# openai/whisper

Hardware: AMD Instinct MI355X
Metric: audio-seconds transcribed per wall-second (large-v3 greedy) (higher is better)
Workload: dtype f16

## Files before the change

whisper_amd/csrc/gemv.hip:

```cpp
#include "common.h"
#include "kernels.h"
#include <stdlib.h>

#ifndef WH_GEMV8_MAX_ROWS
#define WH_GEMV8_MAX_ROWS 24
#endif

namespace {

#define ISSUE_FENCE() asm volatile("" ::: "memory")

constexpr int CS = 4;

__device__ __forceinline__ float4v load_part4(const float* p) { return *(const float4v*)p; }
__device__ __forceinline__ float4v load_part4(const half_t* p) {
  const half4v h = *(const half4v*)p;
  return float4v{(float)h[0], (float)h[1], (float)h[2], (float)h[3]};
}

template <typename T> struct Pack4;
template <> struct Pack4<float> {
  static __device__ __forceinline__ void store(float* p, float a, float b, float c, float d) {
    *(float4v*)p = float4v{a, b, c, d};
  }
// ... 903 lines not shown
      sw = across_groups8_sum(sw);
#pragma unroll
      for (int rt = 0; rt < NRT; ++rt) { s1[rt] = across_groups8_sum(s1[rt]); s2[rt] = across_groups8_sum(s2[rt]); }
      if (lane < 8) {
        wsum[mw][lane] = sw;
#pragma unroll
        for (int rt = 0; rt < NRT; ++rt) { xstat[mw][rt][0][lane] = s1[rt]; xstat[mw][rt][1][lane] = s2[rt]; }
      }
    }
  }
  WH_PROBE_AT(a, wgid, 4);
  __syncthreads();
  WH_PROBE_AT(a, wgid, 5);
#pragma unroll
  for (int j = 0; j < NOUT; ++j) {
    const int o = tid + NT * j;
    const int es = o / (NRT * 64), ert = (o >> 6) % NRT, er = (o >> 3) & 7, ej = o & 7;
    const int en = blockIdx.x * fw + es * 8 + ej;
    const bool on = o < GS * NRT * 64 && ert * 8 + er < R && es * 8 + ej < fw && en < a.N;
    if (on) {
      float v = POST ? 0.f : e_bias[j];
#pragma unroll
      for (int k = 0; k < KS; ++k) v += red[es * KS + k][ert][ej][er];
      const int64_t rr = r0 + ert * 8 + er;
      const int n = en;
      if constexpr (POST) {
        float t1 = 0.f, t2 = 0.f, tw = 0.f;
#pragma unroll
        for (int k = 0; k < KS; ++k) { t1 += xstat[es * KS + k][ert][0][er]; t2 += xstat[es * KS + k][ert][1][er]; tw += wsum[es * KS + k][ej]; }
        const float invK = 1.0f / (float)K;
        const float mc = t1 * invK;
        const float var = fmaxf(__builtin_fmaf(-mc, mc, t2 * invK), 0.f);
        v = __builtin_fmaf(rsqrtf(var + 1e-5f), __builtin_fmaf(-mc, tw, v), e_bias[j]);
      }
      switch (a.epi) {
        case whk::EPI_STORE: ((half_t*)a.y)[a.y_frag ? frag_elem(rr, n, a.N) : rr * a.y_ld + n] = (half_t)v; break;
        case whk::EPI_GELU: ((half_t*)a.y)[a.y_frag ? frag_elem(rr, n, a.N) : rr * a.y_ld + n] = (half_t)gelu_erf(v); break;
        case whk::EPI_F32: ((float*)a.y)[rr * a.y_ld + n] = v; break;
        case whk::EPI_RESID: {
          const float xr = e_res[j] + v;
          a.resid[rr * a.resid_ld + n] = xr;
          if (a.xh) ((half_t*)a.xh)[frag_elem(rr, n, a.N)] = (half_t)fminf(fmaxf(xr - e_cen[j], -65504.f), 65504.f);
        } break;
        case whk::EPI_QKV: {
          const int D = a.D;
          if (n < D) ((half_t*)a.y)[rr * a.y_ld + n] = (half_t)v;
          else {
            const int64_t pos = e_pos - e_lag[j];
            if (n < 2 * D) ((half_t*)a.kcache)[rr * a.cache_bs + pos * D + (n - D)] = (half_t)v;
            else ((half_t*)a.vcache)[rr * a.cache_bs + pos * D + (n - 2 * D)] = (half_t)v;
          }
        } break;
      }
    }
  }
  WH_PROBE_AT(a, wgid, 6);
  if (a.bump && blockIdx.x == 0 && blockIdx.y == 0 && tid == 0) atomicAdd(a.bump, a.bump_by);
  if (a.bump2 && blockIdx.x == 0 && blockIdx.y == 0 && tid == 0) atomicAdd(a.bump2, 1);
}

template <int PRO, int GS, int KS, int CSm, int XW, int NRT>
hipError_t launch_gemv8_nrt(const whk::GemvArgs& a, int fw, hipStream_t stream) {
  constexpr int WAVES = GS * KS + XW;
  static_assert(WAVES <= 16, "at most 1024 threads per workgroup");
  if (fw < 1 || fw > 8 * GS) return hipErrorInvalidValue;
  whk::g_form = WH_FORM_NAME("gemv8/%s/gs%d/ks%d/xw%d/rt%d", PRO == whk::PRO_PLAIN ? "plain" : PRO == whk::PRO_LN ? "LN" : PRO == whk::PRO_LN_POST ? "LNpost" :
                             CSm == 2 ? "combine2" : CSm == 3 ? "combine3" : "combine4", GS, KS, XW, NRT);
  const int nblk = a.K / 64;
  const int nu = (nblk + KS - 1) / KS;
  dim3 grid((a.N + fw - 1) / fw, (a.R + 8 * NRT - 1) / (8 * NRT)), block(WAVES * 64);
  if constexpr (KS == 2) {
    if (nu > 10) return hipErrorInvalidValue;
    hipLaunchKernelGGL((gemv8_kernel<PRO, GS, KS, 10, CSm, XW, NRT>), grid, block, 0, stream, a, fw);
  } else {
    if (nu <= 3) hipLaunchKernelGGL((gemv8_kernel<PRO, GS, KS, 3, CSm, XW, NRT>), grid, block, 0, stream, a, fw);
    else if (nu <= 5) hipLaunchKernelGGL((gemv8_kernel<PRO, GS, KS, 5, CSm, XW, NRT>), grid, block, 0, stream, a, fw);
    else return hipErrorInvalidValue;
  }
  return hipGetLastError();
}

template <int PRO, int GS, int KS, int CSm, int XW>
hipError_t launch_gemv8_cfg(const whk::GemvArgs& a, int fw, hipStream_t stream) {
  if (a.R <= 8) return launch_gemv8_nrt<PRO, GS, KS, CSm, XW, 1>(a, fw, stream);
  if (a.R <= 16) return launch_gemv8_nrt<PRO, GS, KS, CSm, XW, 2>(a, fw, stream);
  if constexpr (GS * KS + XW < 16) {
    if (a.R > 24) return launch_gemv8_nrt<PRO, GS, KS, CSm, XW, 6>(a, fw, stream);
  }
  return launch_gemv8_nrt<PRO, GS, KS, CSm, XW, 3>(a, fw, stream);
}

static int gemv8_fw(int N, int gs) {
  static int ncu = 256;
  int fw = (N + ncu - 1) / ncu;
  if (fw > 8 * gs) fw = 8 * gs;
  if (fw < 4) fw = N < 8 ? N : 8 < 8 * gs ? 8 : 8 * gs;
  return fw;
}

static int gemv8_slots(int N, int pro) {
  const int ngroups = (N + 7) / 8;
  if (pro == whk::PRO_LN) return ngroups >= 600 ? 3 : ngroups >= 400 ? 2 : 1;
  return 1;
}

template <int PRO, int CSm>
hipError_t launch_gemv8_pro(const whk::GemvArgs& a, hipStream_t stream) {
  const int nblk = a.K / 64, gs = gemv8_slots(a.N, PRO), fw = gemv8_fw(a.N, gs);
  if constexpr (PRO == whk::PRO_LN_POST) {
    return a.R <= 16 ? launch_gemv8_nrt<PRO, 1, 4, CSm, 0, 2>(a, fw, stream) : launch_gemv8_nrt<PRO, 1, 4, CSm, 0, 3>(a, fw, stream);
  } else if constexpr (PRO == whk::PRO_PLAIN) {
    if (nblk > 20) {
      whk::GemvArgs b = a;
      b.w_ordered = !WH_DEV_FLAG("WH_GEMV8_W_OPERAND_ORDER");
      return launch_gemv8_cfg<PRO, 1, 16, CSm, 0>(b, fw, stream);
    }
    return launch_gemv8_cfg<PRO, 1, 4, CSm, 0>(a, fw, stream);
  } else {
    if constexpr (PRO == whk::PRO_LN) {
      if (gs == 3 && a.R > 8 && !WH_DEV_FLAG("WH_GEMV8_LN3_KS4")) {
        if (a.R <= 16) return launch_gemv8_nrt<PRO, 3, 2, CSm, 8, 2>(a, fw, stream);
        return launch_gemv8_nrt<PRO, 3, 2, CSm, 8, 3>(a, fw, stream);
      }
      if (gs == 3) return launch_gemv8_cfg<PRO, 3, 4, CSm, 4>(a, fw, stream);
      if (gs == 2) return launch_gemv8_cfg<PRO, 2, 4, CSm, 8>(a, fw, stream);
    }
    return launch_gemv8_cfg<PRO, 1, 4, CSm, 8>(a, fw, stream);
  }
}

bool gemv8_applies(const whk::GemvArgs& a) {
  if (WH_DEV_FLAG("WH_GEMV_DOT2")) return false;
  if (a.variant != 0 || a.R < 1 || a.R > 96 || a.K % 64 != 0) return false;
  const int nblk = a.K / 64;
  if (nblk > 20 && (a.pro != whk::PRO_PLAIN || (nblk + 15) / 16 > 5)) return false;
  if (a.xh && a.epi == whk::EPI_RESID && (a.N % 64 != 0 || !a.xc)) return false;
  if (a.epi == whk::EPI_F32 && a.N > 16384) return false;
  if ((int64_t)a.N * a.K >= (1ll << 31)) return false;
  switch (a.pro) {
    case whk::PRO_PLAIN: return a.x_ld % 8 == 0 && (int64_t)a.R * a.x_ld < (1ll << 30);
    case whk::PRO_LN: return a.ln_folded && a.xf_ld % 4 == 0 && (int64_t)a.R * a.xf_ld < (1ll << 29);
    case whk::PRO_LN_POST: return a.ln_folded && a.R > 8 && a.R <= WH_GEMV8_MAX_ROWS && a.R <= 24 && a.epi != whk::EPI_RESID;
    case whk::PRO_COMBINE:
      return a.K == a.H * 64 && a.H <= 20 && a.splits >= 2 && a.splits <= 4 && (int64_t)a.R * a.H * a.splits * 64 < (1ll << 29);
  }
  return false;
}

hipError_t launch_gemv8(const whk::GemvArgs& a, hipStream_t stream) {
  if (a.pro == whk::PRO_PLAIN) return launch_gemv8_pro<whk::PRO_PLAIN, 1>(a, stream);
  if (a.pro == whk::PRO_LN) return launch_gemv8_pro<whk::PRO_LN, 1>(a, stream);
  if (a.pro == whk::PRO_LN_POST) return a.xh ? launch_gemv8_pro<whk::PRO_LN_POST, 1>(a, stream) : hipErrorInvalidValue;
  if (a.pro == whk::PRO_COMBINE && a.splits == 2) return launch_gemv8_pro<whk::PRO_COMBINE, 2>(a, stream);
  if (a.pro == whk::PRO_COMBINE && a.splits == 3) return launch_gemv8_pro<whk::PRO_COMBINE, 3>(a, stream);
  if (a.pro == whk::PRO_COMBINE && a.splits == 4) return launch_gemv8_pro<whk::PRO_COMBINE, 4>(a, stream);
  return hipErrorInvalidValue;
}

template <int NFT>
__global__ __launch_bounds__(1024) void gemv_rows48_kernel(whk::GemvArgs a) {
  extern __shared__ __attribute__((aligned(16))) char smem[];
  pin_kernargs(a);
  constexpr int WAVES = 16, RT = 48, KSP = WAVES / NFT, J = 5, NU = (40 + KSP - 1) / KSP;
  const int K = a.K, nks = K / 32;
  half_t* xs = (half_t*)smem;
  float* red = (float*)smem;
  const int tid = threadIdx.x, lane = tid & 63;
  const int wave = __builtin_amdgcn_readfirstlane(tid >> 6);
  const int ft = wave % NFT, ksp = wave / NFT;
  const int i16 = lane & 15, g4 = lane >> 4;
  const int n0 = blockIdx.x * (NFT * 16);
  const int R = a.R;

  float4v v[3][J];
#pragma unroll
  for (int i = 0; i < 3; ++i) {
    const int r = wave + WAVES * i;
    const float* src = a.xf + (int64_t)(r < R ? r : 0) * a.xf_ld;
#pragma unroll
    for (int j = 0; j < J; ++j) {
      int k = (j * 64 + lane) * 4; if (k > K - 4) k = K - 4;
      v[i][j] = *(const float4v*)(src + k);
    }
  }
  ISSUE_FENCE();
  half8v w[NU];
  {
    int n = n0 + ft * 16 + i16; if (n > a.N - 1) n = a.N - 1;
    const half_t* base = (const half_t*)a.W + (int64_t)n * K + g4 * 8;
#pragma unroll
    for (int u = 0; u < NU; ++u) {
      int st = ksp + KSP * u; if (st > nks - 1) st = nks - 1;
      w[u] = __builtin_nontemporal_load((const half8v*)(base + st * 32));
    }
  }
  ISSUE_FENCE();
  int e_pos = 0;
  if (a.epi == whk::EPI_QKV) e_pos = load_agent_int(a.d_pos);
  float e_bias[(NFT * 768 + 1023) / 1024];
#pragma unroll
  for (int q = 0; q < (NFT * 768 + 1023) / 1024; ++q) {
    const int o = tid + q * 1024;
    int n = n0 + ((o >> 8) / 3) * 16 + (o & 15); if (n > a.N - 1) n = a.N - 1;
    e_bias[q] = a.bias ? a.bias[n] : 0.f;
  }

  {
    const float invK = 1.0f / (float)K;
#pragma unroll
    for (int i = 0; i < 3; ++i) {
      const int r = wave + WAVES * i;
      float sum = 0.f;
#pragma unroll
      for (int j = 0; j < J; ++j) {
        const float t = (v[i][j][0] + v[i][j][1]) + (v[i][j][2] + v[i][j][3]);
        sum += ((j * 64 + lane) * 4 < K) ? t : 0.f;
      }
      const float mean = wave_sum(sum) * invK;
      float ss = 0.f;
#pragma unroll
      for (int j = 0; j < J; ++j) {
        if ((j * 64 + lane) * 4 < K) {
#pragma unroll
          for (int e = 0; e < 4; ++e) { const float d = v[i][j][e] - mean; ss = __builtin_fmaf(d, d, ss); }
        }
      }
      const float rstd = r < R ? rsqrtf(wave_sum(ss) * invK + 1e-5f) : 0.f;
      half_t* xr = xs + (size_t)r * K;
#pragma unroll
      for (int j = 0; j < J; ++j) {
        const int k = (j * 64 + lane) * 4;
        if (k < K)
          Pack4<half_t>::store(xr + ((((k >> 3) ^ (r & 15)) << 3) | (k & 7)), (v[i][j][0] - mean) * rstd,
                               (v[i][j][1] - mean) * rstd, (v[i][j][2] - mean) * rstd, (v[i][j][3] - mean) * rstd);
      }
    }
  }
  __syncthreads();

  float4v acc[3];
#pragma unroll
  for (int rt = 0; rt < 3; ++rt) acc[rt] = float4v{0.f, 0.f, 0.f, 0.f};
#pragma unroll
  for (int u = 0; u < NU; ++u) {
    const int st = ksp + KSP * u;
    if (st < nks) {
#pragma unroll
      for (int rt = 0; rt < 3; ++rt) {
        const half8v xf = *(const half8v*)(xs + (size_t)(rt * 16 + i16) * K + (((st * 4 + g4) ^ i16) << 3));
        acc[rt] = __builtin_amdgcn_mfma_f32_16x16x32_f16(w[u], xf, acc[rt], 0, 0, 0);
      }
    }
  }
  __syncthreads();
#pragma unroll
  for (int rt = 0; rt < 3; ++rt) *(float4v*)(red + ((((ksp * NFT + ft) * 3 + rt) * 16 + i16) * 16 + g4 * 4)) = acc[rt];
  __syncthreads();

#pragma unroll
  for (int q = 0; q < (NFT * 768 + 1023) / 1024; ++q) {
    const int o = tid + q * 1024;
    if (o >= NFT * 768) continue;
    const int f = o & 15, j = (o >> 4) & 15, rt = (o >> 8) % 3, oft = (o >> 8) / 3;
    const int row = rt * 16 + j, n = n0 + oft * 16 + f;
    if (row >= R || n >= a.N) continue;
    float val = e_bias[q];
#pragma unroll
    for (int k = 0; k < KSP; ++k) val += red[((((k * NFT + oft) * 3 + rt) * 16 + j) * 16) + f];
    const int64_t rr = row;
    switch (a.epi) {
      case whk::EPI_STORE: ((half_t*)a.y)[rr * a.y_ld + n] = (half_t)val; break;
      case whk::EPI_GELU: ((half_t*)a.y)[rr * a.y_ld + n] = (half_t)gelu_erf(val); break;
      case whk::EPI_QKV: {
        const int D = a.D;
        if (n < D) ((half_t*)a.y)[rr * a.y_ld + n] = (half_t)val;
        else {
          const int64_t pos = e_pos - (a.lag ? a.lag[row] : 0);
          if (n < 2 * D) ((half_t*)a.kcache)[rr * a.cache_bs + pos * D + (n - D)] = (half_t)val;
          else ((half_t*)a.vcache)[rr * a.cache_bs + pos * D + (n - 2 * D)] = (half_t)val;
        }
      } break;
      default: break;
    }
  }
  if (a.bump && blockIdx.x == 0 && tid == 0) atomicAdd(a.bump, a.bump_by);
  if (a.bump2 && blockIdx.x == 0 && tid == 0) atomicAdd(a.bump2, 1);
}

bool rows48_applies(const whk::GemvArgs& a) {
  return !WH_DEV_FLAG("WH_NO_ROWS48") && a.R > WH_GEMV8_MAX_ROWS && a.R <= 48 && a.pro == whk::PRO_LN && a.ln_folded &&
         a.K % 256 == 0 && a.K <= 1280 && a.N >= 2048 && a.variant <= 0 &&
         (a.epi == whk::EPI_STORE || a.epi == whk::EPI_GELU || a.epi == whk::EPI_QKV);
}

hipError_t launch_rows48(const whk::GemvArgs& a, hipStream_t stream) {
  whk::g_form = "rows48";
  const size_t lds = (size_t)48 * a.K * 2 > 49152 ? (size_t)48 * a.K * 2 : 49152;
  static whk::LdsAttr attr2;
  { hipError_t e = whk::raise_dynamic_lds(attr2, (const void*)gemv_rows48_kernel<2>, 160 * 1024); if (e != hipSuccess) return e; }
  hipLaunchKernelGGL((gemv_rows48_kernel<2>), dim3((a.N + 31) / 32), dim3(1024), lds, stream, a);
  return hipGetLastError();
}

__global__ __launch_bounds__(1024) void gemv_rows48_stream_kernel(whk::GemvArgs a) {
  extern __shared__ __attribute__((aligned(16))) char smem[];
  pin_kernargs(a);
  constexpr int WAVES = 16, J = 5, NB = 20;
  const int K = a.K, nks = K / 32;
  half_t* xs = (half_t*)smem;
  float* gb = (float*)(smem + (size_t)48 * K * 2);
  const int tid = threadIdx.x, lane = tid & 63;
  const int wave = __builtin_amdgcn_readfirstlane(tid >> 6);
  const int i16 = lane & 15, g4 = lane >> 4;
  const int R = a.R;
  const int ntiles = (a.N + 15) / 16;

  float4v v[3][J];
#pragma unroll
  for (int i = 0; i < 3; ++i) {
    const int r = wave + WAVES * i;
    const float* src = a.xf + (int64_t)(r < R ? r : 0) * a.xf_ld;
#pragma unroll
    for (int j = 0; j < J; ++j) {
      int k = (j * 64 + lane) * 4; if (k > K - 4) k = K - 4;
      v[i][j] = *(const float4v*)(src + k);
    }
  }
  for (int k = tid * 4; k < K; k += 4096) {
    *(float4v*)(gb + k) = *(const float4v*)(a.ln_w + k);
    *(float4v*)(gb + K + k) = *(const float4v*)(a.ln_b + k);
  }
  __syncthreads();
  {
    const float invK = 1.0f / (float)K;
#pragma unroll
    for (int i = 0; i < 3; ++i) {
      const int r = wave + WAVES * i;
      float sum = 0.f;
#pragma unroll
      for (int j = 0; j < J; ++j) {
        const float t = (v[i][j][0] + v[i][j][1]) + (v[i][j][2] + v[i][j][3]);
        sum += ((j * 64 + lane) * 4 < K) ? t : 0.f;
      }
      const float mean = wave_sum(sum) * invK;
      float ss = 0.f;
#pragma unroll
      for (int j = 0; j < J; ++j) {
        if ((j * 64 + lane) * 4 < K) {
#pragma unroll
          for (int e = 0; e < 4; ++e) { const float d = v[i][j][e] - mean; ss = __builtin_fmaf(d, d, ss); }
        }
      }
      const float rstd = rsqrtf(wave_sum(ss) * invK + 1e-5f);
      half_t* xr = xs + (size_t)r * K;
#pragma unroll
      for (int j = 0; j < J; ++j) {
        const int k = (j * 64 + lane) * 4;
        if (k < K) {
          const float4v w4 = *(const float4v*)(gb + k), b4 = *(const float4v*)(gb + K + k);
          half_t* dst = xr + ((((k >> 3) ^ (r & 15)) << 3) | (k & 7));
          if (r < R)
            Pack4<half_t>::store(dst, (v[i][j][0] - mean) * rstd * w4[0] + b4[0], (v[i][j][1] - mean) * rstd * w4[1] + b4[1],
                                 (v[i][j][2] - mean) * rstd * w4[2] + b4[2], (v[i][j][3] - mean) * rstd * w4[3] + b4[3]);
          else
            Pack4<half_t>::store(dst, 0.f, 0.f, 0.f, 0.f);
        }
      }
    }
  }
  __syncthreads();

  for (int tile = blockIdx.x * WAVES + wave; tile < ntiles; tile += gridDim.x * WAVES) {
    int n = tile * 16 + i16; if (n > a.N - 1) n = a.N - 1;
    const half_t* base = (const half_t*)a.W + (int64_t)n * K + g4 * 8;
    float4v acc[3];
#pragma unroll
    for (int rt = 0; rt < 3; ++rt) acc[rt] = float4v{0.f, 0.f, 0.f, 0.f};
    for (int st0 = 0; st0 < nks; st0 += NB) {
      half8v w[NB];
#pragma unroll
      for (int u = 0; u < NB; ++u) {
        int st = st0 + u; if (st > nks - 1) st = nks - 1;
        w[u] = __builtin_nontemporal_load((const half8v*)(base + st * 32));
      }
#pragma unroll
      for (int u = 0; u < NB; ++u) {
        const int st = st0 + u;
        if (st < nks) {
#pragma unroll
          for (int rt = 0; rt < 3; ++rt) {
            const half8v xf = *(const half8v*)(xs + (size_t)(rt * 16 + i16) * K + (((st * 4 + g4) ^ i16) << 3));
            acc[rt] = __builtin_amdgcn_mfma_f32_16x16x32_f16(w[u], xf, acc[rt], 0, 0, 0);
          }
        }
      }
    }
#pragma unroll
    for (int rt = 0; rt < 3; ++rt) {
      const int row = rt * 16 + i16;
      if (row < R) {
        float* y = (float*)a.y + (int64_t)row * a.y_ld + tile * 16 + g4 * 4;
#pragma unroll
        for (int e = 0; e < 4; ++e)
          if (tile * 16 + g4 * 4 + e < a.N) y[e] = acc[rt][e];
      }
    }
  }
  if (a.bump && blockIdx.x == 0 && tid == 0) atomicAdd(a.bump, a.bump_by);
  if (a.bump2 && blockIdx.x == 0 && tid == 0) atomicAdd(a.bump2, 1);
}

bool rows48_stream_applies(const whk::GemvArgs& a) {
  return !WH_DEV_FLAG("WH_NO_ROWS48") && a.R > 16 && a.R <= 48 && a.pro == whk::PRO_LN && a.epi == whk::EPI_F32 && !a.bias &&
         a.K % 256 == 0 && a.K <= 1280 && a.N >= 16384 && a.variant <= 0;
}

hipError_t launch_rows48_stream(const whk::GemvArgs& a, hipStream_t stream) {
  whk::g_form = "rows48_stream";
  const size_t lds = (size_t)48 * a.K * 2 + (size_t)2 * a.K * 4;
  static whk::LdsAttr attr;
  { hipError_t e = whk::raise_dynamic_lds(attr, (const void*)gemv_rows48_stream_kernel, 160 * 1024); if (e != hipSuccess) return e; }
  const int ntiles = (a.N + 15) / 16;
  int wgs = (ntiles + 15) / 16;
  if (wgs > 256) wgs = 256;
  hipLaunchKernelGGL(gemv_rows48_stream_kernel, dim3(wgs), dim3(1024), lds, stream, a);
  return hipGetLastError();
}

template <typename T, int MS>
__global__ __launch_bounds__(256) void merge_partials_kernel(const T* __restrict__ part_o, const float* __restrict__ part_ml,
                                                             int S, int R, int H, T* __restrict__ out, int64_t o_ld, int o_frag) {
  const int i = blockIdx.x * 256 + threadIdx.x;
  if (i >= R * H * 16) return;
  const int r = i / (H * 16), rem = i - r * (H * 16);
  const int h = rem >> 4, d4 = rem & 15;
  const int64_t pb = (int64_t)r * H + h, ps = (int64_t)R * H;
  float2v ml[MS];
  float4v o[MS];
#pragma unroll
  for (int s = 0; s < MS; ++s) {
    const int sc = s < S ? s : S - 1;
    ml[s] = *(const float2v*)(part_ml + (pb + sc * ps) * 2);
    o[s] = load_part4(part_o + (pb + sc * ps) * 64 + d4 * 4);
  }
  float M = WH_NEG_INF;
#pragma unroll
  for (int s = 0; s < MS; ++s) { if (s >= S) ml[s] = float2v{WH_NEG_INF, 0.f}; M = fmaxf(M, ml[s][0]); }
  float w[MS], den = 0.f;
#pragma unroll
  for (int s = 0; s < MS; ++s) {
    w[s] = (ml[s][0] == WH_NEG_INF) ? 0.f : __expf(ml[s][0] - M);
    den = __builtin_fmaf(w[s], ml[s][1], den);
  }
  const float inv = 1.0f / den;
  float4v num = {0.f, 0.f, 0.f, 0.f};
#pragma unroll
  for (int s = 0; s < MS; ++s) {
    const float f = w[s] * ml[s][1] * inv;
    num[0] = __builtin_fmaf(f, o[s][0], num[0]); num[1] = __builtin_fmaf(f, o[s][1], num[1]);
    num[2] = __builtin_fmaf(f, o[s][2], num[2]); num[3] = __builtin_fmaf(f, o[s][3], num[3]);
  }
  Pack4<T>::store(out + (o_frag ? frag_elem(r, h * 64 + d4 * 4, H * 64) : (int64_t)r * o_ld + h * 64 + d4 * 4), num[0], num[1], num[2], num[3]);
}

enum class Family { refuse, gemv8, rows48, rows48_stream, rows16_mf, rt4, rt8 };

Family pick_family(const whk::GemvArgs& a, int dtype) {
  if (a.R <= 0) return Family::refuse;
  if (a.xc && a.pro != whk::PRO_LN && !(a.xh && a.epi == whk::EPI_RESID)) return Family::refuse;
  if (a.x_frag || a.y_frag || a.pro == whk::PRO_LN_POST || a.xh || a.xc) return dtype == 1 && a.R <= WH_GEMV8_MAX_ROWS && gemv8_applies(a) ? Family::gemv8 : Family::refuse;
  if (dtype != 1) return a.R <= 4 || a.K > 3072 ? Family::rt4 : Family::rt8;
  if (rows48_applies(a)) return Family::rows48;
  if (rows48_stream_applies(a)) return Family::rows48_stream;
  const bool rows16 = a.R > 8 && a.variant <= 0 && a.K % 128 == 0 && a.K <= 5120 && (a.K / 32 <= 40 || a.pro == whk::PRO_PLAIN);
  if ((a.R <= WH_GEMV8_MAX_ROWS || !rows16) && gemv8_applies(a)) return Family::gemv8;
  if (a.R <= 4) return Family::rt4;
  if (rows16) return Family::rows16_mf;
  return Family::rt8;
}

}

namespace whk {

thread_local const char* g_form = "";

hipError_t launch_gemv(const GemvArgs& a, int dtype, hipStream_t stream) {
  const Family f = pick_family(a, dtype);
  if (dtype == 1) {
    switch (f) {
      case Family::gemv8: return launch_gemv8(a, stream);
      case Family::rows48: return launch_rows48(a, stream);
      case Family::rows48_stream: return launch_rows48_stream(a, stream);
      case Family::rt4: return launch_rt<half_t, 4>(a, stream);
      case Family::rows16_mf: return launch_rows16_mf<half_t>(a, stream);
      case Family::rt8: return launch_rt<half_t, 8>(a, stream);
      case Family::refuse: break;
    }
  } else if (f == Family::rt4 || f == Family::rt8) {
    return f == Family::rt4 ? launch_rt<float, 4>(a, stream) : launch_rt<float, 8>(a, stream);
  }
  return hipErrorInvalidValue;
}

const char* gemv_family(const GemvArgs& a, int dtype) {
  static const char* const names[] = {"", "gemv8", "rows48", "rows48_stream", "rows16_mf", "rt4", "rt8"};
  return names[(int)pick_family(a, dtype)];
}

bool gemv8_will_run(int R, int N, int K, int pro) {
  GemvArgs a = {};
  a.pro = pro; a.R = R; a.N = N; a.K = K; a.x_ld = a.xf_ld = K; a.ln_folded = 1; a.splits = 2; a.H = K / 64;
  a.epi = EPI_STORE; a.y_frag = 1;
  return pick_family(a, 1) == Family::gemv8;
}

bool gemv8_ln_post_pays(int R, int N, int K) {
  GemvArgs a = {};
  a.pro = PRO_LN_POST; a.R = R; a.N = N; a.K = K; a.ln_folded = 1; a.epi = EPI_STORE;
  return pick_family(a, 1) == Family::gemv8 && gemv8_slots(N, PRO_LN) == 1 && gemv8_will_run(R, N, K, PRO_LN);
}

hipError_t launch_merge_partials(const void* part_o, const float* part_ml, int splits, int R, int H, void* out,
                                 int64_t o_ld, int dtype, hipStream_t stream, int o_frag) {
  if (splits < 1 || splits > DEC_ATTN_MAX_SPLITS || R <= 0 || H <= 0) return hipErrorInvalidValue;
  const int n = R * H * 16;
  const dim3 grid((n + 255) / 256), block(256);
  g_form = dtype == 1 ? (splits <= 4 ? "merge<half,4>" : "merge<half,16>") : (splits <= 4 ? "merge<float,4>" : "merge<float,16>");
  if (dtype == 1) {
    if (splits <= 4)
      hipLaunchKernelGGL((merge_partials_kernel<half_t, 4>), grid, block, 0, stream, (const half_t*)part_o, part_ml, splits, R, H, (half_t*)out, o_ld, o_frag);
    else
      hipLaunchKernelGGL((merge_partials_kernel<half_t, DEC_ATTN_MAX_SPLITS>), grid, block, 0, stream, (const half_t*)part_o, part_ml, splits, R, H, (half_t*)out, o_ld, o_frag);
  } else {
    if (splits <= 4)
      hipLaunchKernelGGL((merge_partials_kernel<float, 4>), grid, block, 0, stream, (const float*)part_o, part_ml, splits, R, H, (float*)out, o_ld, o_frag);
    else
      hipLaunchKernelGGL((merge_partials_kernel<float, DEC_ATTN_MAX_SPLITS>), grid, block, 0, stream, (const float*)part_o, part_ml, splits, R, H, (float*)out, o_ld, o_frag);
  }
  return hipGetLastError();
}

}
```

Before: 1177.

## Pipeline weight loads across tiles and specialize rows48 stream GEMV on K and row tiles

Templates the LN-fused rows48 streaming GEMV on K/256 and on the number of 16-row tiles (2 when R<=32), so loops are fully unrolled and one row tile of MFMA work is skipped for smaller batches. Weight loads are double-buffered in blocks of 8: the first tile's weights are requested before the LayerNorm prologue, and the next tile's weights are prefetched right after the current tile's output stores. The grid becomes up to 256 workgroups with one tile per wave interleaved, and LDS addressing is precomputed per lane. The cost is more template instantiations and higher register pressure from the two weight buffers.

```diff
diff --git a/whisper_amd/csrc/gemv.hip b/whisper_amd/csrc/gemv.hip
--- a/whisper_amd/csrc/gemv.hip
+++ b/whisper_amd/csrc/gemv.hip
@@ -1229,39 +1229,61 @@
   return hipGetLastError();
 }
 
+template <int NB, int U0 = 0, int U1 = NB>
+__device__ __forceinline__ void rows48_stream_request(half8v (&w)[NB], const half_t* base, int b) {
+#pragma unroll
+  for (int u = U0; u < U1; ++u) w[u] = __builtin_nontemporal_load((const half8v*)(base + (b * NB + u) * 32));
+}
+
+template <int NT, int NBT>
 __global__ __launch_bounds__(1024) void gemv_rows48_stream_kernel(whk::GemvArgs a) {
   extern __shared__ __attribute__((aligned(16))) char smem[];
   pin_kernargs(a);
-  constexpr int WAVES = 16, J = 5, NB = 20;
-  const int K = a.K, nks = K / 32;
+  constexpr int WAVES = 16, J = 5, NB = 8;
+  constexpr int K = 256 * NBT;
+  constexpr int E1 = NT == 2 ? 2 : 0;
   half_t* xs = (half_t*)smem;
-  float* gb = (float*)(smem + (size_t)48 * K * 2);
+  float* gb = (float*)(smem + (size_t)(16 * NT) * K * 2);
   const int tid = threadIdx.x, lane = tid & 63;
   const int wave = __builtin_amdgcn_readfirstlane(tid >> 6);
   const int i16 = lane & 15, g4 = lane >> 4;
   const int R = a.R;
   const int ntiles = (a.N + 15) / 16;
-
-  float4v v[3][J];
-#pragma unroll
-  for (int i = 0; i < 3; ++i) {
+  const int lap = gridDim.x * WAVES;
+  int tile = wave * gridDim.x + blockIdx.x;
+  auto wbase = [&](int t) {
+    int n = t * 16 + i16; if (n > a.N - 1) n = a.N - 1;
+    if (t >= ntiles) n = 0;
+    return (const half_t*)a.W + (int64_t)n * K + g4 * 8;
+  };
+
+  float4v v[NT][J];
+#pragma unroll
+  for (int i = 0; i < NT; ++i) {
     const int r = wave + WAVES * i;
     const float* src = a.xf + (int64_t)(r < R ? r : 0) * a.xf_ld;
 #pragma unroll
     for (int j = 0; j < J; ++j) {
       int k = (j * 64 + lane) * 4; if (k > K - 4) k = K - 4;
+      if (r >= R) k = 0;
       v[i][j] = *(const float4v*)(src + k);
     }
   }
-  for (int k = tid * 4; k < K; k += 4096) {
-    *(float4v*)(gb + k) = *(const float4v*)(a.ln_w + k);
-    *(float4v*)(gb + K + k) = *(const float4v*)(a.ln_b + k);
-  }
+  const int gk = tid * 4 < K ? tid * 4 : K - 4;
+  const float4v gw = *(const float4v*)(a.ln_w + gk), gbt = *(const float4v*)(a.ln_b + gk);
+  ISSUE_FENCE();
+  half8v w[2][NB];
+  const half_t* base = wbase(tile);
+  rows48_stream_request(w[0], base, 0);
+  if (NBT > 1) rows48_stream_request<NB, 0, E1>(w[1], base, 1);
+  ISSUE_FENCE();
+  if (tid * 4 < K) { *(float4v*)(gb + tid * 4) = gw; *(float4v*)(gb + K + tid * 4) = gbt; }
   __syncthreads();
   {
+#pragma clang fp contract(off)
     const float invK = 1.0f / (float)K;
 #pragma unroll
-    for (int i = 0; i < 3; ++i) {
+    for (int i = 0; i < NT; ++i) {
       const int r = wave + WAVES * i;
       float sum = 0.f;
 #pragma unroll
@@ -1278,7 +1300,7 @@
           for (int e = 0; e < 4; ++e) { const float d = v[i][j][e] - mean; ss = __builtin_fmaf(d, d, ss); }
         }
       }
-      const float rstd = rsqrtf(wave_sum(ss) * invK + 1e-5f);
+      const float rstd = rsqrtf(__builtin_fmaf(wave_sum(ss), invK, 1e-5f));
       half_t* xr = xs + (size_t)r * K;
 #pragma unroll
       for (int j = 0; j < J; ++j) {
@@ -1286,44 +1308,46 @@
         if (k < K) {
           const float4v w4 = *(const float4v*)(gb + k), b4 = *(const float4v*)(gb + K + k);
           half_t* dst = xr + ((((k >> 3) ^ (r & 15)) << 3) | (k & 7));
-          if (r < R)
-            Pack4<half_t>::store(dst, (v[i][j][0] - mean) * rstd * w4[0] + b4[0], (v[i][j][1] - mean) * rstd * w4[1] + b4[1],
-                                 (v[i][j][2] - mean) * rstd * w4[2] + b4[2], (v[i][j][3] - mean) * rstd * w4[3] + b4[3]);
-          else
-            Pack4<half_t>::store(dst, 0.f, 0.f, 0.f, 0.f);
-        }
-      }
-    }
-  }
+          float o[4];
+#pragma unroll
+          for (int e = 0; e < 4; ++e) {
+            o[e] = __builtin_fmaf((v[i][j][e] - mean) * rstd, w4[e], b4[e]);
+            asm volatile("" : "+v"(o[e]));
+            if (r >= R) o[e] = 0.f;
+          }
+          Pack4<half_t>::store(dst, o[0], o[1], o[2], o[3]);
+        }
+      }
+    }
+  }
+  if (NBT > 1) rows48_stream_request<NB, E1, NB>(w[1], base, 1);
+  ISSUE_FENCE();
   __syncthreads();
 
-  for (int tile = blockIdx.x * WAVES + wave; tile < ntiles; tile += gridDim.x * WAVES) {
-    int n = tile * 16 + i16; if (n > a.N - 1) n = a.N - 1;
-    const half_t* base = (const half_t*)a.W + (int64_t)n * K + g4 * 8;
-    float4v acc[3];
-#pragma unroll
-    for (int rt = 0; rt < 3; ++rt) acc[rt] = float4v{0.f, 0.f, 0.f, 0.f};
-    for (int st0 = 0; st0 < nks; st0 += NB) {
-      half8v w[NB];
+  const half_t* xrow[4];
+#pragma unroll
+  for (int s = 0; s < 4; ++s) xrow[s] = xs + (size_t)i16 * K + ((((s ^ (i16 >> 2)) << 2) | (g4 ^ (i16 & 3))) << 3);
+
+  while (tile < ntiles) {
+    float4v acc[NT];
+#pragma unroll
+    for (int rt = 0; rt < NT; ++rt) acc[rt] = float4v{0.f, 0.f, 0.f, 0.f};
+#pragma unroll
+    for (int b = 0; b < NBT; ++b) {
+      if (b >= 1 && b + 1 < NBT) rows48_stream_request(w[(b + 1) & 1], base, b + 1);
+      ISSUE_FENCE();
 #pragma unroll
       for (int u = 0; u < NB; ++u) {
-        int st = st0 + u; if (st > nks - 1) st = nks - 1;
-        w[u] = __builtin_nontemporal_load((const half8v*)(base + st * 32));
-      }
-#pragma unroll
-      for (int u = 0; u < NB; ++u) {
-        const int st = st0 + u;
-        if (st < nks) {
-#pragma unroll
-          for (int rt = 0; rt < 3; ++rt) {
-            const half8v xf = *(const half8v*)(xs + (size_t)(rt * 16 + i16) * K + (((st * 4 + g4) ^ i16) << 3));
-            acc[rt] = __builtin_amdgcn_mfma_f32_16x16x32_f16(w[u], xf, acc[rt], 0, 0, 0);
-          }
-        }
-      }
-    }
-#pragma unroll
-    for (int rt = 0; rt < 3; ++rt) {
+        const int st = b * NB + u;
+#pragma unroll
+        for (int rt = 0; rt < NT; ++rt) {
+          const half8v xf = *(const half8v*)(xrow[st & 3] + (size_t)(rt * 16) * K + (st >> 2) * 128);
+          acc[rt] = __builtin_amdgcn_mfma_f32_16x16x32_f16(w[b & 1][u], xf, acc[rt], 0, 0, 0);
+        }
+      }
+    }
+#pragma unroll
+    for (int rt = 0; rt < NT; ++rt) {
       const int row = rt * 16 + i16;
       if (row < R) {
         float* y = (float*)a.y + (int64_t)row * a.y_ld + tile * 16 + g4 * 4;
@@ -1332,6 +1356,12 @@
           if (tile * 16 + g4 * 4 + e < a.N) y[e] = acc[rt][e];
       }
     }
+    tile += lap;
+    if (tile < ntiles) {
+      base = wbase(tile);
+      rows48_stream_request(w[0], base, 0);
+      if (NBT > 1) rows48_stream_request(w[1], base, 1);
+    }
   }
   if (a.bump && blockIdx.x == 0 && tid == 0) atomicAdd(a.bump, a.bump_by);
   if (a.bump2 && blockIdx.x == 0 && tid == 0) atomicAdd(a.bump2, 1);
@@ -1342,16 +1372,28 @@
          a.K % 256 == 0 && a.K <= 1280 && a.N >= 16384 && a.variant <= 0;
 }
 
+template <int NT, int NBT>
+hipError_t launch_rows48_stream_as(const whk::GemvArgs& a, hipStream_t stream) {
+  const size_t lds = (size_t)(16 * NT) * a.K * 2 + (size_t)2 * a.K * 4;
+  static whk::LdsAttr attr;
+  { hipError_t e = whk::raise_dynamic_lds(attr, (const void*)gemv_rows48_stream_kernel<NT, NBT>, 160 * 1024); if (e != hipSuccess) return e; }
+  const int ntiles = (a.N + 15) / 16;
+  const int wgs = ntiles < 256 ? ntiles : 256;
+  hipLaunchKernelGGL((gemv_rows48_stream_kernel<NT, NBT>), dim3(wgs), dim3(1024), lds, stream, a);
+  return hipGetLastError();
+}
+
 hipError_t launch_rows48_stream(const whk::GemvArgs& a, hipStream_t stream) {
   whk::g_form = "rows48_stream";
-  const size_t lds = (size_t)48 * a.K * 2 + (size_t)2 * a.K * 4;
-  static whk::LdsAttr attr;
-  { hipError_t e = whk::raise_dynamic_lds(attr, (const void*)gemv_rows48_stream_kernel, 160 * 1024); if (e != hipSuccess) return e; }
-  const int ntiles = (a.N + 15) / 16;
-  int wgs = (ntiles + 15) / 16;
-  if (wgs > 256) wgs = 256;
-  hipLaunchKernelGGL(gemv_rows48_stream_kernel, dim3(wgs), dim3(1024), lds, stream, a);
-  return hipGetLastError();
+  const bool two = a.R <= 32;
+  switch (a.K / 256) {
+    case 1: return two ? launch_rows48_stream_as<2, 1>(a, stream) : launch_rows48_stream_as<3, 1>(a, stream);
+    case 2: return two ? launch_rows48_stream_as<2, 2>(a, stream) : launch_rows48_stream_as<3, 2>(a, stream);
+    case 3: return two ? launch_rows48_stream_as<2, 3>(a, stream) : launch_rows48_stream_as<3, 3>(a, stream);
+    case 4: return two ? launch_rows48_stream_as<2, 4>(a, stream) : launch_rows48_stream_as<3, 4>(a, stream);
+    case 5: return two ? launch_rows48_stream_as<2, 5>(a, stream) : launch_rows48_stream_as<3, 5>(a, stream);
+    default: return hipErrorInvalidValue;
+  }
 }
 
 template <typename T, int MS>
```

Result: no change. 1181 (median of 6 runs) (+0.4%).
